# filixi/TCP-stack

Hardware: AMD Instinct MI355X
Metric: GiB/s device-resident TCP checksum over batched segments; % HBM roofline (higher is better)
Workload: dtype u16; 1 GPU; C2: 1M x 1460-B payload (1492-B images), fixed stride, device-resident; images_per_gpu=1048576, image_bytes=1492, bytes_per_gpu=1564475392, parallelism=shard1 (independent per-GPU batches, no collective)

## Files before the change

tcp-stack_amd/csrc/tcpck_device.h:

```cpp
#pragma once

#include <hip/hip_runtime.h>
#include <stdint.h>

#include "tcpck_internal.h"

namespace tcpck {
namespace dev {

using u32x4 = __attribute__((ext_vector_type(4))) unsigned int;

constexpr int kBlock = 256;
constexpr int kWavesPerBlock = kBlock / 64;

template <typename Kernel>
inline uint32_t resident_blocks_per_cu(Kernel kernel) {
  int nb = 0;
  if (hipOccupancyMaxActiveBlocksPerMultiprocessor(&nb, kernel, kBlock, 0) != hipSuccess || nb < 1) nb = 1;
  return static_cast<uint32_t>(nb);
}

inline uint32_t oversub_for(uint32_t requested, uint64_t bytes, uint64_t resident_waves, uint32_t max_m,
                            uint32_t min_run = 4u << 10) {
  if (requested) return requested;
  const uint64_t q = bytes / (resident_waves * min_run + 1);
  uint32_t m = 1;
  while (2 * m <= max_m && 2 * m <= q) m *= 2;
  return m;
}

__device__ __forceinline__ uint64_t align16_rel(const uint8_t *arena, uint64_t off) {
  const uint64_t mis = reinterpret_cast<uint64_t>(arena) & 15u;
  return ((off + mis) & ~uint64_t{15}) - mis;
}

__device__ __forceinline__ uint64_t align128_rel(const uint8_t *arena, uint64_t off) {
  const uint64_t mis = reinterpret_cast<uint64_t>(arena) & 127u;
  return ((off + mis) & ~uint64_t{127}) - mis;
}

__device__ __forceinline__ u32x4 load16_nt(const uint8_t *p) {
  return __builtin_nontemporal_load(reinterpret_cast<const u32x4 *>(p));
}

__device__ __forceinline__ uint32_t word_mask(int32_t lo, int32_t hi) {
  return ((1u << (hi >> 1)) - 1u) & ~((1u << (lo >> 1)) - 1u);
}

__device__ __forceinline__ uint32_t dword_mask(uint32_t wm, int j) {
  const uint32_t t = (wm >> (2 * j)) & 3u;
  return ((t & 1u) ? 0x0000FFFFu : 0u) | ((t & 2u) ? 0xFFFF0000u : 0u);
}

__device__ __forceinline__ u32x4 apply_mask(u32x4 w, uint32_t wm) {
  w.x &= dword_mask(wm, 0);
  w.y &= dword_mask(wm, 1);
  w.z &= dword_mask(wm, 2);
  w.w &= dword_mask(wm, 3);
  return w;
}

__device__ __forceinline__ uint32_t ref_add(uint32_t acc, uint32_t w) { return acc + w + (w >> 16); }

__device__ __forceinline__ uint32_t ref_chunk_sum(u32x4 w) {
  return ref_add(ref_add(ref_add(w.x + (w.x >> 16), w.y), w.z), w.w);
}

__device__ __forceinline__ uint32_t dot2_u16(uint32_t w, uint32_t acc) {
  uint32_t r;
  asm("v_dot2_u32_u16 %0, %1, %2, %3" : "=v"(r) : "v"(w), "s"(0x00010001u), "v"(acc));
  return r;
}
__device__ __forceinline__ uint32_t ref_chunk_sum_dot(u32x4 w) {
  return dot2_u16(w.w, dot2_u16(w.z, dot2_u16(w.y, dot2_u16(w.x, 0u))));
}

__device__ __forceinline__ __amdgpu_buffer_rsrc_t make_rsrc(const void *p, uint32_t bytes) {
  const uint64_t a = reinterpret_cast<uint64_t>(p);
  const uint32_t lo = static_cast<uint32_t>(__builtin_amdgcn_readfirstlane(static_cast<int>(a)));
  const uint32_t hi = static_cast<uint32_t>(__builtin_amdgcn_readfirstlane(static_cast<int>(a >> 32)));
  const int n = __builtin_amdgcn_readfirstlane(static_cast<int>(bytes));
  void *u = reinterpret_cast<void *>((static_cast<uint64_t>(hi) << 32) | lo);
  return __builtin_amdgcn_make_buffer_rsrc(u, 0, n, 0x00020000);
}
__device__ __forceinline__ void store16_field(__amdgpu_buffer_rsrc_t r, uint32_t voff, uint16_t v) {
  __builtin_amdgcn_raw_buffer_store_b16(v, r, static_cast<int>(voff), 0, 16);
}

__device__ __forceinline__ uint32_t n2h_selector(uint32_t j) {
  return j == 3 ? 0x02030001u : ((j == 2 || j >= 6) ? 0x02030100u : 0x00010203u);
}
__device__ __forceinline__ uint32_t n2h_dword(uint32_t h, uint32_t sel) {
  return __builtin_amdgcn_perm(h, h, sel);
}

__device__ __forceinline__ u32x4 load16_buf_nt(__amdgpu_buffer_rsrc_t r, uint32_t voff, uint32_t soff) {
  typedef unsigned v4u __attribute__((ext_vector_type(4)));
  const v4u v = __builtin_amdgcn_raw_buffer_load_b128(r, static_cast<int>(voff), static_cast<int>(soff), 2);
  return u32x4{v.x, v.y, v.z, v.w};
}

__device__ __forceinline__ uint32_t rfc_add(uint32_t acc, uint32_t w) {
  const uint32_t s = acc + w;
  return s + (s < w ? 1u : 0u);
}

template <int MODE>
__device__ __forceinline__ uint32_t accumulate(uint32_t acc, uint32_t w) {
  if constexpr (MODE == kRef) {
    return ref_add(acc, w);
  } else {
    return rfc_add(acc, w);
  }
}

template <int MODE>
__device__ __forceinline__ uint32_t fold_lane(uint32_t acc) {
  if constexpr (MODE == kRef) {
    return acc & 0xFFFFu;
  } else {
    acc = (acc & 0xFFFFu) + (acc >> 16);
    return (acc & 0xFFFFu) + (acc >> 16);
  }
}

template <int MODE>
__device__ __forceinline__ uint16_t finish(uint32_t sum) {
  if constexpr (MODE == kRef) {
    return static_cast<uint16_t>(~sum);
  } else {
    sum = (sum & 0xFFFFu) + (sum >> 16);
    sum = (sum & 0xFFFFu) + (sum >> 16);
    return static_cast<uint16_t>(~sum);
  }
}

template <int G>
__device__ __forceinline__ uint32_t group_sum(uint32_t x) {
#pragma unroll
  for (int m = G / 2; m >= 1; m >>= 1) x += __shfl_xor(x, m, 64);
  return x;
}

__device__ __forceinline__ uint32_t wave_inclusive_scan(uint32_t x) {
  x += __builtin_amdgcn_update_dpp(0, x, 0x111, 0xF, 0xF, false);
  x += __builtin_amdgcn_update_dpp(0, x, 0x112, 0xF, 0xF, false);
  x += __builtin_amdgcn_update_dpp(0, x, 0x114, 0xF, 0xF, false);
  x += __builtin_amdgcn_update_dpp(0, x, 0x118, 0xF, 0xF, false);
  x += __builtin_amdgcn_update_dpp(0, x, 0x142, 0xA, 0xF, false);
  x += __builtin_amdgcn_update_dpp(0, x, 0x143, 0xC, 0xF, false);
  return x;
}

__device__ __forceinline__ uint32_t read_lane(uint32_t x, uint32_t lane) {
  return static_cast<uint32_t>(__builtin_amdgcn_readlane(static_cast<int>(x), static_cast<int>(lane)));
}

__device__ __forceinline__ uint64_t read_lane64(uint64_t x, uint32_t lane) {
  const uint32_t lo = read_lane(static_cast<uint32_t>(x), lane);
  const uint32_t hi = read_lane(static_cast<uint32_t>(x >> 32), lane);
  return (static_cast<uint64_t>(hi) << 32) | lo;
}

template <bool EXACT = false>
__device__ __forceinline__ uint32_t words_before(uint32_t r, uint32_t x, uint32_t y, uint32_t z, uint32_t w) {
  const uint32_t nw = r >> 1;
  uint32_t h = 0;
  auto both = [](uint32_t d) -> uint32_t { return EXACT ? (d & 0xFFFFu) + (d >> 16) : d + (d >> 16); };
  if (nw >= 2) h += both(x);
  if (nw >= 4) h += both(y);
  if (nw >= 6) h += both(z);
  if (nw & 1) {
    const uint32_t d = nw == 1 ? x : (nw == 3 ? y : (nw == 5 ? z : w));
    h += d & 0xFFFFu;
  }
  return h;
}

template <int U, int MODE>
__device__ __forceinline__ uint32_t wave_image_sum(const uint8_t *arena, uint64_t start, uint32_t len,
                                                   bool exclude_field) {
  const uint32_t lane = threadIdx.x & 63;
  const uint64_t a0 = align16_rel(arena, start);
  const uint8_t *p0 = arena + a0;
  const int32_t lead = static_cast<int32_t>(start - a0);
  const int64_t span64 = lead + static_cast<int64_t>(len);
  const uint32_t nch = static_cast<uint32_t>((span64 + 15) >> 4);
  const int64_t field = exclude_field ? lead + 28 : -64;
  uint32_t acc = 0;
  for (uint32_t i0 = lane; i0 < nch; i0 += 64 * U) {
    u32x4 v[U];
#pragma unroll
    for (int u = 0; u < U; ++u) {
      const uint32_t i = i0 + u * 64;
      v[u] = load16_nt(p0 + 16 * static_cast<uint64_t>(i < nch ? i : nch - 1));
    }
#pragma unroll
    for (int u = 0; u < U; ++u) {
      const int64_t rel = 16 * static_cast<int64_t>(i0 + u * 64);
      const int32_t lo = static_cast<int32_t>(min(max(lead - rel, int64_t{0}), int64_t{16}));
      const int32_t hi = static_cast<int32_t>(min(max(span64 - rel, int64_t{0}), int64_t{16}));
      uint32_t wm = word_mask(lo, hi);
      const int64_t fb = field - rel;
      if (fb >= 0 && fb < 16) wm &= ~(1u << (fb >> 1));
      u32x4 w = v[u];
      if (wm != 0xFFu) w = apply_mask(w, wm);
      acc = accumulate<MODE>(acc, w.x);
      acc = accumulate<MODE>(acc, w.y);
      acc = accumulate<MODE>(acc, w.z);
      acc = accumulate<MODE>(acc, w.w);
    }
    if (MODE == kRfc1071) acc = fold_lane<MODE>(acc);
  }
  return group_sum<64>(fold_lane<MODE>(acc));
}

__device__ __forceinline__ uint64_t find_first_ge(const uint64_t *offsets, uint64_t base, uint64_t count, uint64_t target) {
  const uint32_t lane = threadIdx.x & 63;
  uint64_t lo = 0, hi = count;
  while (hi - lo > 64) {
    const uint64_t step = (hi - lo + 63) / 64;
    const uint64_t idx = lo + lane * step;
    const bool below = idx < hi && offsets[idx] - base < target;
    const uint32_t c = __popcll(__ballot(below));
    const uint64_t nlo = c ? lo + (c - 1) * step + 1 : lo;
    const uint64_t nhi = min(hi, lo + c * step);
    lo = nlo;
    hi = nhi;
  }
  const uint64_t idx = lo + lane;
  const bool below = idx < hi && offsets[idx] - base < target;
  return lo + __popcll(__ballot(below));
}

__device__ __forceinline__ void find_two(const uint64_t *offsets, uint64_t base, uint64_t count, uint64_t t0,
                                         uint64_t t1, uint64_t &r0, uint64_t &r1) {
  const uint32_t lane = threadIdx.x & 63;
  uint64_t lo[2] = {0, 0}, hi[2] = {count, count};
  const uint64_t t[2] = {t0, t1};
  while (hi[0] - lo[0] > 64 || hi[1] - lo[1] > 64) {
    uint64_t step[2], idx[2], v[2];
#pragma unroll
    for (int i = 0; i < 2; ++i) {
      step[i] = hi[i] - lo[i] > 64 ? (hi[i] - lo[i] + 63) / 64 : 1;
      idx[i] = lo[i] + lane * step[i];
      v[i] = idx[i] < hi[i] ? offsets[idx[i]] : 0;
    }
#pragma unroll
    for (int i = 0; i < 2; ++i) {
      if (hi[i] - lo[i] <= 64) continue;
      const bool below = idx[i] < hi[i] && v[i] - base < t[i];
      const uint32_t c = __popcll(__ballot(below));
      const uint64_t nlo = c ? lo[i] + (c - 1) * step[i] + 1 : lo[i];
      hi[i] = min(hi[i], lo[i] + c * step[i]);
      lo[i] = nlo;
    }
  }
  uint64_t v[2];
#pragma unroll
  for (int i = 0; i < 2; ++i) {
    const uint64_t idx = lo[i] + lane;
    v[i] = idx < hi[i] ? offsets[idx] : 0;
  }
  const bool b0 = lo[0] + lane < hi[0] && v[0] - base < t0;
  const bool b1 = lo[1] + lane < hi[1] && v[1] - base < t1;
  r0 = lo[0] + __popcll(__ballot(b0));
  r1 = lo[1] + __popcll(__ballot(b1));
}

__device__ __forceinline__ void count_split(uint64_t wid, uint64_t q, uint64_t r, uint64_t &kb, uint64_t &ke) {
  kb = wid * q + (wid < r ? wid : r);
  ke = kb + q + (wid < r ? 1u : 0u);
}

__device__ __forceinline__ uint32_t xcd_block(uint32_t b, uint32_t nb) {
  const uint32_t q = nb >> 3, r = nb & 7u, x = b & 7u;
  return (x < r ? x * (q + 1) : r * (q + 1) + (x - r) * q) + (b >> 3);
}

__device__ __forceinline__ uint32_t xcd_chunk_block(uint32_t b, uint32_t nb, uint32_t lc) {
  const uint32_t full = (nb >> (3 + lc)) << (3 + lc);
  if (b >= full) return b;
  const uint32_t i = b >> 3;
  return ((((i >> lc) << 3) + (b & 7u)) << lc) + (i & ((1u << lc) - 1u));
}

constexpr uint32_t kOrderDefault = 0xFFu;
constexpr uint32_t kOrderXcd = 0xFEu;
__device__ __forceinline__ uint32_t ordered_block(uint32_t b, uint32_t nb, uint32_t lc) {
  if (lc == kOrderDefault) return b;
  if (lc == kOrderXcd) return xcd_block(b, nb);
  return xcd_chunk_block(b, nb, lc);
}


}
}
```

tcp-stack_amd/csrc/tcpck_vvstream.hip:

```cpp
#include <type_traits>

#include "tcpck_device.h"
#include "tcpck_internal.h"

namespace tcpck {

namespace {

using dev::kBlock;
using dev::kWavesPerBlock;
using dev::u32x4;

constexpr uint32_t kRound = 256;
constexpr uint32_t kRing = 512;
constexpr uint32_t kMirror = 64;

struct VVArgs {
  uint8_t *arena;
  const uint64_t *offsets;
  const uint32_t *lengths;
  uint64_t base;
  uint64_t count;
  void *out;
  uint64_t per_wave, rem;
  uint32_t stride;
  uint32_t len;
  uint32_t order;
  uint32_t keep_first;
  uint32_t defer_field;
  uint64_t *dbg;
};

#ifdef TCPCK_PROBE
__device__ __forceinline__ uint64_t stamp_after(uint32_t dep) {
  uint64_t t;
  asm volatile("s_memrealtime %0\n\ts_waitcnt lgkmcnt(0)" : "=s"(t) : "v"(dep));
  return t;
}
#endif

__device__ __forceinline__ u32x4 zero_word(u32x4 w, uint32_t wi) {
  const uint32_t keep = (wi & 1u) ? 0x0000FFFFu : 0xFFFF0000u;
  const uint32_t di = wi >> 1;
  w.x &= di == 0 ? keep : 0xFFFFFFFFu;
  w.y &= di == 1 ? keep : 0xFFFFFFFFu;
  w.z &= di == 2 ? keep : 0xFFFFFFFFu;
  w.w &= di == 3 ? keep : 0xFFFFFFFFu;
  return w;
}

[[maybe_unused]] __device__ __forceinline__ u32x4 put_word(u32x4 w, uint32_t wi, uint32_t v) {
  const uint32_t sh = (wi & 1u) << 4;
  const uint32_t m = ~(0xFFFFu << sh), x = (v & 0xFFFFu) << sh;
  const uint32_t di = wi >> 1;
  w.x = di == 0 ? (w.x & m) | x : w.x;
  w.y = di == 1 ? (w.y & m) | x : w.y;
  w.z = di == 2 ? (w.z & m) | x : w.z;
  w.w = di == 3 ? (w.w & m) | x : w.w;
  return w;
}

[[maybe_unused]] __device__ __forceinline__ void store16_chunk_wt(__amdgpu_buffer_rsrc_t r, uint32_t voff, u32x4 v) {
  typedef unsigned v4u __attribute__((ext_vector_type(4)));
  __builtin_amdgcn_raw_buffer_store_b128(v4u{v.x, v.y, v.z, v.w}, r, static_cast<int>(voff), 0, 19);
}

template <int U, int OP, int SPLIT, int LAYOUT, bool KEEP = false, int MODE = kRef, bool BLK = false>
__global__ void __launch_bounds__(kBlock) vvstream_kernel(VVArgs a) {
  constexpr bool FIXED = LAYOUT != 0;
  constexpr bool GAP = LAYOUT == 2;
  static_assert(!BLK || (OP == kFill && !GAP && MODE == kRef && !KEEP), "BLK: reference-mode FILL, no gaps");
  constexpr uint32_t kMinFill = BLK ? 64u : 30u;
  __shared__ u32x4 s_blk[kWavesPerBlock][BLK ? 4 : 1];
  __shared__ uint32_t s_end[kWavesPerBlock][FIXED ? 1 : kRing + kMirror];
  __shared__ __attribute__((aligned(16))) uint32_t s_pre[kWavesPerBlock][MODE == kRef ? 256 : 512];
  __shared__ uint32_t s_fld[kWavesPerBlock][OP == kFill ? 64 : 1];
  const uint32_t lane = threadIdx.x & 63;
  const uint32_t wv = static_cast<uint32_t>(__builtin_amdgcn_readfirstlane(static_cast<int>(threadIdx.x >> 6)));
  const uint64_t W = static_cast<uint64_t>(gridDim.x) * kWavesPerBlock;
  const uint32_t bid = dev::ordered_block(blockIdx.x, gridDim.x, a.order);
  const uint64_t wid = static_cast<uint64_t>(bid) * kWavesPerBlock + wv;
  const uint64_t N = a.count;
#ifdef TCPCK_PROBE
  const uint64_t t_start = a.dbg ? __builtin_amdgcn_s_memrealtime() : 0;
  uint64_t t_desc = 0, t_first = 0;
#endif
  const uint32_t S = a.stride;
  const uint32_t L = FIXED ? a.len : 0u;
  uint64_t kb, ke;
  if (FIXED || SPLIT == 1) {
    dev::count_split(wid, a.per_wave, a.rem, kb, ke);
  } else {
    const uint64_t first = a.offsets[0] - a.base;
    const uint64_t total = a.offsets[N - 1] - a.base + a.lengths[N - 1] - first;
    const uint64_t q = total / W, rm = total % W;
    dev::find_two(a.offsets, a.base, N, first + q * wid + rm * wid / W,
                  first + q * (wid + 1) + rm * (wid + 1) / W, kb, ke);
    if (wid == 0) kb = 0;
    if (wid + 1 == W) ke = N;
  }
  if (kb >= ke) return;

  uint64_t s0, s1;
  if constexpr (FIXED) {
    s0 = kb * S;
    s1 = (ke - 1) * S + L;
  } else {
    s0 = a.offsets[kb] - a.base;
    s1 = a.offsets[ke - 1] - a.base + a.lengths[ke - 1];
  }
  uint8_t *const arena = a.arena;
  const uint64_t A0 = dev::align128_rel(arena, s0);
  const uint32_t nimg = static_cast<uint32_t>(ke - kb);
  const uint32_t nv = GAP ? 2 * nimg : nimg;
  bool bad = !(s1 >= s0 && s1 - A0 < (uint64_t{1} << 31));
#ifdef TCPCK_PROBE
  if (a.dbg) t_desc = stamp_after(static_cast<uint32_t>(s1 - A0));
#endif

  auto store = [&](uint64_t k, uint32_t sum, uint64_t start) {
    const uint16_t c = dev::finish<MODE>(sum);
    if constexpr (OP == kVerify) {
      static_cast<uint8_t *>(a.out)[k] = (c == 0) ? 1 : 0;
    } else {
      if (a.out) static_cast<uint16_t *>(a.out)[k] = c;
      if (OP == kFill) *reinterpret_cast<uint16_t *>(arena + start + 28) = c;
    }
  };
  auto store_rel = [&](uint64_t k, uint32_t sum, uint32_t start_rel, __amdgpu_buffer_rsrc_t r) {
    const uint16_t c = dev::finish<MODE>(sum);
    if constexpr (OP == kVerify) {
      static_cast<uint8_t *>(a.out)[k] = (c == 0) ? 1 : 0;
    } else {
      if (a.out) static_cast<uint16_t *>(a.out)[k] = c;
      if (OP == kFill && !a.defer_field) dev::store16_field(r, start_rel + 28, c);
    }
  };

  if (!bad) {
    const uint32_t lead = static_cast<uint32_t>(s0 - A0);
    const uint32_t span = static_cast<uint32_t>(s1 - A0);
    const uint32_t nsteps = (span + 1023) >> 10;
    const uint32_t last_chunk = span > 0 ? (span - 1) >> 4 : 0;
    int64_t blo = 0, bhi = 0;
    uint32_t extent = (last_chunk + 1) << 4;
    if constexpr (BLK) {
      const uint64_t b0 = FIXED ? 0 : a.offsets[0] - a.base;
      const uint64_t b1 = FIXED ? (N - 1) * S + L : a.offsets[N - 1] - a.base + a.lengths[N - 1];
      blo = static_cast<int64_t>(b0) - static_cast<int64_t>(A0);
      bhi = static_cast<int64_t>(b1) - static_cast<int64_t>(A0);
      const int64_t want = min(static_cast<int64_t>((span + 63u) & ~63u), bhi & ~int64_t{15});
      if (want > static_cast<int64_t>(extent)) extent = static_cast<uint32_t>(want);
    }
    const auto rsrc = dev::make_rsrc(arena + A0, extent);
    auto whole = [&](uint32_t b) { return static_cast<int64_t>(b) >= blo && static_cast<int64_t>(b) + 64 <= bhi; };
    uint32_t stage_f = 0;
    auto load_step = [&](uint32_t st) -> u32x4 {
      if constexpr (KEEP) {
        typedef unsigned v4u __attribute__((ext_vector_type(4)));
        const v4u v = __builtin_amdgcn_raw_buffer_load_b128(rsrc, static_cast<int>(lane << 4), static_cast<int>(st << 10), 0);
        return u32x4{v.x, v.y, v.z, v.w};
      } else {
        return dev::load16_buf_nt(rsrc, lane << 4, st << 10);
      }
    };
    uint32_t *ring_end = s_end[wv];
    u32x4 *pre4 = reinterpret_cast<u32x4 *>(s_pre[wv]);
    const uint16_t *pre16 = reinterpret_cast<const uint16_t *>(s_pre[wv]);
    uint32_t *fld = s_fld[wv];
    if constexpr (OP == kFill) {
      fld[lane] = 0;
      __builtin_amdgcn_wave_barrier();
    }

    uint32_t carry = 0, p_last = 0, jn = 0, fj = 0;
    uint32_t e_last = lead;
    u32x4 ring[U];
#pragma unroll
    for (int u = 0; u < U; ++u) {
      if (u == 0 && a.keep_first && (lane < 8 || a.keep_first == 2)) {
        typedef unsigned v4u __attribute__((ext_vector_type(4)));
        const v4u v = __builtin_amdgcn_raw_buffer_load_b128(rsrc, static_cast<int>(lane << 4), 0, 0);
        ring[0] = u32x4{v.x, v.y, v.z, v.w};
      } else {
        ring[u] = load_step(static_cast<uint32_t>(u));
      }
    }

    const uint32_t *lens = FIXED ? nullptr : a.lengths + kb;
    auto load_round = [&](uint32_t r, uint32_t (&d)[4]) {
#pragma unroll
      for (int i = 0; i < 4; ++i) {
        const uint32_t j = r * kRound + 4 * lane + i;
        d[i] = j < nimg ? lens[j] : 0u;
      }
    };
    uint32_t loaded = FIXED ? nv : 0;
    uint32_t pos = lead;
    bool short_fill = false;
    bool al4 = (lead & 3u) == 0 && (!FIXED || ((S & 3u) == 0 && (!GAP || (L & 3u) == 0)));
    auto fill_round = [&]() {
      const uint32_t r = loaded / kRound;
      uint32_t d[4];
      load_round(r, d);
      al4 = al4 && __ballot(((d[0] | d[1] | d[2] | d[3]) & 3u) != 0) == 0;
      if constexpr (MODE == kRfc1071) {
        bad = bad || __ballot((d[0] | d[1] | d[2] | d[3]) >= (1u << 17)) != 0;
      }
      const uint32_t e1 = d[0], e2 = e1 + d[1], e3 = e2 + d[2], e4 = e3 + d[3];
      const uint32_t incl = dev::wave_inclusive_scan(e4);
      const uint32_t ex = pos + incl - e4;
      if constexpr (OP == kFill) {
        const uint32_t jb = r * kRound + 4 * lane;
        bool sh = false;
#pragma unroll
        for (int i = 0; i < 4; ++i) sh |= (jb + i < nimg) && d[i] < kMinFill;
        short_fill |= __ballot(sh) != 0;
      }
      const uint32_t jb = r * kRound + 4 * lane;
      const uint32_t v0 = jb < nimg ? ex + e1 : ~0u, v1 = jb + 1 < nimg ? ex + e2 : ~0u;
      const uint32_t v2 = jb + 2 < nimg ? ex + e3 : ~0u, v3 = jb + 3 < nimg ? ex + e4 : ~0u;
      const uint32_t si = (r * kRound) % kRing + 4 * lane;
      ring_end[si] = v0;
      ring_end[si + 1] = v1;
      ring_end[si + 2] = v2;
      ring_end[si + 3] = v3;
      if (si < kMirror) {
        ring_end[kRing + si] = v0;
        ring_end[kRing + si + 1] = v1;
        ring_end[kRing + si + 2] = v2;
        ring_end[kRing + si + 3] = v3;
      }
      pos = pos + dev::read_lane(incl, 63);
      loaded += kRound;
      if (loaded >= nimg) {
        const uint32_t sn = loaded % kRing + lane;
        ring_end[sn] = ~0u;
        if (sn < kMirror) ring_end[kRing + sn] = ~0u;
      }
      __builtin_amdgcn_wave_barrier();
    };
    if constexpr (!FIXED) {
      fill_round();
      if constexpr (OP == kFill) {
        if (nimg > kRound) {
          uint32_t sum = 0;
          bool sh = false;
          for (uint32_t j = lane; j < nimg; j += 64) {
            const uint32_t l = lens[j];
            sum += l;
            sh |= l < kMinFill || (MODE == kRfc1071 && l >= (1u << 17));
          }
          short_fill = short_fill || __ballot(sh) != 0;
          bad = bad || short_fill || lead + dev::group_sum<64>(sum) != span;
        } else {
          bad = bad || short_fill || pos != span;
        }
      }
    } else {
      if constexpr (OP == kFill) bad = L < kMinFill;
    }
    auto end_of = [&](uint32_t j) -> uint32_t {
      if constexpr (GAP) {
        return lead + (j >> 1) * S + (j & 1u) * L;
      } else if constexpr (FIXED) {
        return lead + (j + 1) * S;
      } else {
        return ring_end[j % kRing];
      }
    };
    auto ends_at = [&](uint32_t jn0) -> uint32_t {
      if constexpr (FIXED) {
        const uint32_t j = jn0 + lane;
        return j < nv ? end_of(j) : ~0u;
      } else {
        return ring_end[jn0 % kRing + lane];
      }
    };

    auto stream_run = [&](auto al4_tag) {
      constexpr bool AL4 = decltype(al4_tag)::value;
      for (uint32_t g = 0; g < nsteps && !bad; g += U) {
  #pragma unroll
        for (int u = 0; u < U; ++u) {
          const uint32_t st = g + u;
          const uint32_t sb = st << 10;
          const uint32_t c = sb + (lane << 4);
          u32x4 w = ring[u];
          const u32x4 raw = w;
          if (sb == 0 || sb + 1024 > span) {
            const int32_t lo = min(max(static_cast<int32_t>(lead) - static_cast<int32_t>(c), 0), 16);
            const int32_t hi = min(max(static_cast<int32_t>(span) - static_cast<int32_t>(c), 0), 16);
            w = dev::apply_mask(w, dev::word_mask(lo, hi));
          }
          if (!FIXED && jn + 66 > loaded && loaded < nimg) fill_round();
          uint32_t j = jn + lane;
          uint32_t e = ends_at(jn);
          if constexpr (OP == kFill) {
            const uint32_t i = fj + lane;
            uint32_t f;
            if constexpr (FIXED)
              f = lead + i * S + 28;
            else
              f = (i == 0 ? lead : (i < nimg ? end_of(i - 1) : span)) + 28;
            const bool inf = i < nimg && f < sb + 1024;
            const uint64_t bf = __ballot(inf);
            if (bf) {
              if (inf) fld[(f - sb) >> 4] = ((f & 15u) >> 1) + 1u;
              __builtin_amdgcn_wave_barrier();
              const uint32_t q = fld[lane];
              if (q) {
                fld[lane] = 0u;
                w = zero_word(w, q - 1u);
              }
              __builtin_amdgcn_wave_barrier();
              fj += static_cast<uint32_t>(__popcll(bf));
            }
          }
          const uint32_t q1 = dev::dot2_u16(w.x, 0u);
          const uint32_t q2 = dev::dot2_u16(w.y, q1);
          const uint32_t q3 = dev::dot2_u16(w.z, q2);
          const uint32_t tot = dev::dot2_u16(w.w, q3);
#ifdef TCPCK_PROBE
          if (a.dbg && st == 0) t_first = stamp_after(tot);
#endif
          const uint32_t incl = dev::wave_inclusive_scan(tot);
          bool table = false;
          for (;;) {
            const bool inb = e < sb + 1024;
            const uint64_t bal = __ballot(inb);
            if (!bal) break;
            if (!table) {
              const uint32_t p0 = carry + incl - tot;
              const uint32_t b1 = p0 + q1, b2 = p0 + q2, b3 = p0 + q3;
              if constexpr (AL4) {
                pre4[lane] = u32x4{p0, b1, b2, b3};
              } else if constexpr (MODE == kRfc1071) {
                pre4[2 * lane] = u32x4{p0, p0 + (w.x & 0xFFFFu), b1, b1 + (w.y & 0xFFFFu)};
                pre4[2 * lane + 1] = u32x4{b2, b2 + (w.z & 0xFFFFu), b3, b3 + (w.w & 0xFFFFu)};
              } else
                pre4[lane] = u32x4{__builtin_amdgcn_perm(p0 + w.x, p0, 0x05040100u),
                                   __builtin_amdgcn_perm(b1 + w.y, b1, 0x05040100u),
                                   __builtin_amdgcn_perm(b2 + w.z, b2, 0x05040100u),
                                   __builtin_amdgcn_perm(b3 + w.w, b3, 0x05040100u)};
              __builtin_amdgcn_wave_barrier();
              table = true;
            }
            const uint32_t cnt = static_cast<uint32_t>(__popcll(bal));
            const uint32_t off = min(e - sb, 1022u);
            const uint32_t P = AL4 ? s_pre[wv][off >> 2]
                                   : (MODE == kRfc1071 ? s_pre[wv][off >> 1] : static_cast<uint32_t>(pre16[off >> 1]));
            const uint32_t pprev = static_cast<uint32_t>(
                __builtin_amdgcn_update_dpp(static_cast<int>(p_last), static_cast<int>(P), 0x138, 0xF, 0xF, false));
            if constexpr (OP == kFill) {
              const uint32_t el = static_cast<uint32_t>(
                  __builtin_amdgcn_update_dpp(static_cast<int>(e_last), static_cast<int>(e), 0x138, 0xF, 0xF, false));
              const uint32_t start = lane == 0 ? e_last : el;
              if constexpr (BLK) {
                if (inb) {
                  const uint16_t c = dev::finish<MODE>(P - pprev);
                  if (a.out) static_cast<uint16_t *>(a.out)[kb + j] = c;
                  const uint32_t f = start + 28;
                  if (f >= sb) {
                    fld[(f - sb) >> 4] = 0x80000000u | (((f & 15u) >> 1) << 16) | c;
                  } else if (whole(f & ~63u)) {
                    reinterpret_cast<uint16_t *>(s_blk[wv])[(f & 63u) >> 1] = c;
                  } else {
                    dev::store16_field(rsrc, f, c);
                  }
                }
              } else if (inb && (!GAP || (j & 1u))) {
                store_rel(kb + (GAP ? j >> 1 : j), P - pprev, start, rsrc);
              }
            } else {
              if (inb && (!GAP || (j & 1u))) store(kb + (GAP ? j >> 1 : j), P - pprev, 0);
            }
            p_last = dev::read_lane(P, cnt - 1);
            e_last = dev::read_lane(e, cnt - 1);
            jn += cnt;
            if (cnt < 64) break;
            if (!FIXED && jn + 66 > loaded && loaded < nimg) fill_round();
            j = jn + lane;
            e = ends_at(jn);
          }
          if constexpr (BLK) {
            __builtin_amdgcn_wave_barrier();
            if (stage_f != 0 && stage_f < e_last) {
              if (lane < 4 && whole(stage_f & ~63u)) store16_chunk_wt(rsrc, (stage_f & ~63u) + 16 * lane, s_blk[wv][lane]);
              stage_f = 0;
            }
            const uint32_t v = fld[lane];
            const uint64_t bv = __ballot(v != 0);
            if (bv) {
              const uint32_t cb = sb + ((lane & ~3u) << 4);
              if ((bv >> (lane & ~3u)) & 0xFull) {
                if (whole(cb))
                  store16_chunk_wt(rsrc, sb + (lane << 4), v ? put_word(raw, (v >> 16) & 7u, v) : raw);
                else if (v)
                  dev::store16_field(rsrc, sb + (lane << 4) + (((v >> 16) & 7u) << 1), static_cast<uint16_t>(v));
              }
              if (v) fld[lane] = 0u;
            }
            if (jn < nv) {
              const uint32_t f = e_last + 28;
              if (f >= sb && f < sb + 1024) {
                const uint32_t cb = f & ~63u;
                if (((sb + (lane << 4)) & ~63u) == cb) s_blk[wv][lane & 3u] = raw;
                stage_f = f;
              }
            }
          }
          __builtin_amdgcn_wave_barrier();
          carry += dev::read_lane(incl, 63);
          ring[u] = load_step(st + U);
        }
      }
    };
    if (al4 && (FIXED || loaded >= nimg))
      stream_run(std::true_type{});
    else
      stream_run(std::false_type{});
    if constexpr (!FIXED) bad = bad || pos != span || loaded < nimg;
    if (BLK && !bad && jn < nv) {
      const uint16_t c = dev::finish<MODE>(carry - p_last);
      if (lane == 0 && a.out) static_cast<uint16_t *>(a.out)[kb + jn] = c;
      const uint32_t f = e_last + 28;
      if (whole(f & ~63u)) {
        if (lane == 0) reinterpret_cast<uint16_t *>(s_blk[wv])[(f & 63u) >> 1] = c;
        __builtin_amdgcn_wave_barrier();
        if (lane < 4) store16_chunk_wt(rsrc, (f & ~63u) + 16 * lane, s_blk[wv][lane]);
      } else if (lane == 0) {
        dev::store16_field(rsrc, f, c);
      }
      jn = nv - 1 == jn ? nv : jn;
    }
    if (!bad && jn < nv) {
      const uint32_t rem = nv - jn;
      for (uint32_t i = lane; i < rem; i += 64) {
        const uint32_t v = jn + i;
        if (!GAP || (v & 1u)) store_rel(kb + (GAP ? v >> 1 : v), i == 0 ? carry - p_last : 0u, i == 0 ? e_last : span, rsrc);
      }
      jn = nv;
    }
    bad = bad || jn != nv;
  }
#ifdef TCPCK_PROBE
  if (a.dbg && lane == 0) {
    uint32_t hw_id, xcc_id;
    asm volatile("s_getreg_b32 %0, hwreg(HW_REG_HW_ID)" : "=s"(hw_id));
    asm volatile("s_getreg_b32 %0, hwreg(HW_REG_XCC_ID)" : "=s"(xcc_id));
    uint64_t *d = a.dbg + 8 * wid;
    d[0] = t_start;
    d[1] = t_desc;
    d[2] = t_first;
    d[3] = __builtin_amdgcn_s_memrealtime();
    d[4] = hw_id | (static_cast<uint64_t>(xcc_id) << 32);
    d[5] = ke - kb;
    d[6] = s1 - s0;
    d[7] = 0;
  }
#endif
  if (bad) {
    for (uint64_t k = kb; k < ke; ++k) {
      const uint64_t start = FIXED ? k * S : a.offsets[k] - a.base;
      const uint32_t len = FIXED ? L : a.lengths[k];
      if (OP == kFill && len < 30) continue;
      const uint32_t sum = dev::wave_image_sum<2, MODE>(arena, start, len, OP == kFill);
      if (lane == 0) store(k, sum, start);
    }
  }
}

template <int U, int OP, int SPLIT, int LAYOUT, bool KEEP = false, int MODE = kRef, bool BLK = false>
hipError_t launch_one(const RunArgs &s, uint32_t oversub, int flags, uint32_t num_cus, hipStream_t stream) {
  static const uint32_t per_cu = dev::resident_blocks_per_cu(vvstream_kernel<U, OP, SPLIT, LAYOUT, KEEP, MODE, BLK>);
  const uint64_t resident = static_cast<uint64_t>(per_cu) * num_cus;
  uint64_t blocks = resident * (oversub ? oversub : 1);
  const uint64_t need = (s.count + kWavesPerBlock - 1) / kWavesPerBlock;
  if (blocks > need) blocks = need;
  if (blocks == 0) return hipSuccess;
  VVArgs a{};
  a.arena = s.arena;
  a.offsets = s.offsets;
  a.lengths = s.lengths;
  a.base = s.base;
  a.count = s.count;
  a.out = s.out;
  a.per_wave = s.count / (blocks * kWavesPerBlock);
  a.rem = s.count % (blocks * kWavesPerBlock);
  a.stride = static_cast<uint32_t>(s.stride);
  a.len = s.len;
  a.order = (flags & 8) ? 4u : dev::kOrderDefault;
  a.keep_first = (flags & 16) ? ((flags & 256) ? 2u : 1u) : 0u;
  a.defer_field = (flags & 64) ? 1u : 0u;
  a.dbg = s.dbg;
  hipLaunchKernelGGL((vvstream_kernel<U, OP, SPLIT, LAYOUT, KEEP, MODE, BLK>), dim3(static_cast<uint32_t>(blocks)),
                     dim3(kBlock), 0, stream, a);
  return hipGetLastError();
}

template <int U, int SPLIT, int LAYOUT>
hipError_t dispatch(int op, const RunArgs &a, uint32_t oversub, int flags, uint32_t num_cus, hipStream_t s) {
  if (a.mode != kRef) {
    switch (op) {
      case kChecksum: return launch_one<U, kChecksum, SPLIT, LAYOUT, false, kRfc1071>(a, oversub, flags, num_cus, s);
      case kVerify: return launch_one<U, kVerify, SPLIT, LAYOUT, false, kRfc1071>(a, oversub, flags, num_cus, s);
      case kFill: return launch_one<U, kFill, SPLIT, LAYOUT, false, kRfc1071>(a, oversub, flags, num_cus, s);
      default: return hipErrorInvalidValue;
    }
  }
  switch (op) {
    case kChecksum: return launch_one<U, kChecksum, SPLIT, LAYOUT>(a, oversub, flags, num_cus, s);
    case kVerify: return launch_one<U, kVerify, SPLIT, LAYOUT>(a, oversub, flags, num_cus, s);
    case kFill:
#ifdef TCPCK_PROBE
      if constexpr (LAYOUT != 2)
        if (flags & 128) return launch_one<U, kFill, SPLIT, LAYOUT, false, kRef, true>(a, oversub, flags, num_cus, s);
#endif
      return (flags & 32) ? launch_one<U, kFill, SPLIT, LAYOUT, true>(a, oversub, flags, num_cus, s)
                          : launch_one<U, kFill, SPLIT, LAYOUT>(a, oversub, flags, num_cus, s);
    default: return hipErrorInvalidValue;
  }
}

}

hipError_t launch_vvstream(int op, int variant, bool fixed, const RunArgs &a, uint32_t num_cus,
                           hipStream_t stream) {
  if (a.count == 0) return hipSuccess;
  if (fixed && (a.len == 0 || a.stride < a.len || a.stride > (1u << 24))) return hipErrorInvalidValue;
  const bool gap = fixed && a.stride != a.len;
  const uint64_t bytes = fixed ? a.count * a.stride : a.total_bytes;
  uint32_t m = a.oversub ? a.oversub : 1;
  int flags = variant & 248;
  if ((flags & 64) && (op != kFill || !a.out)) return hipErrorInvalidValue;
#ifdef TCPCK_PROBE
  if ((flags & 128) && (op != kFill || a.mode != kRef || gap || (flags & 96))) return hipErrorInvalidValue;
#else
  if (flags & 128) return hipErrorInvalidValue;
#endif
  variant &= 7;
#ifdef TCPCK_PROBE
  if (variant == 5) {
    variant = 4;
    flags |= 256;
  }
#endif
  int u8 = (variant & 1);
  int split = variant >= 2 ? 1 : 0;
  if (variant == 4) {
    m = dev::oversub_for(a.oversub, bytes, static_cast<uint64_t>(num_cus) * 32, 1024, 8u << 10);
    u8 = m >= 32;
    if (op == kFill && !fixed && !(flags & 224)) {
      m = dev::oversub_for(a.oversub, bytes, static_cast<uint64_t>(num_cus) * 32, 1024, 4u << 10);
      u8 = false;
    }
    split = m >= 4;
  } else {
#ifdef TCPCK_PROBE
    if (variant > 4 || variant < 0) return hipErrorInvalidValue;
#else
    return hipErrorInvalidValue;
#endif
  }
  if (gap) return u8 ? dispatch<8, 1, 2>(op, a, m, flags, num_cus, stream) : dispatch<4, 1, 2>(op, a, m, flags, num_cus, stream);
  if (fixed) return u8 ? dispatch<8, 1, 1>(op, a, m, flags, num_cus, stream) : dispatch<4, 1, 1>(op, a, m, flags, num_cus, stream);
  if (split) return u8 ? dispatch<8, 1, 0>(op, a, m, flags, num_cus, stream) : dispatch<4, 1, 0>(op, a, m, flags, num_cus, stream);
  return u8 ? dispatch<8, 0, 0>(op, a, m, flags, num_cus, stream) : dispatch<4, 0, 0>(op, a, m, flags, num_cus, stream);
}

}
```

Measured before the change: 6912 GiB/s.

## Unify AL4 stream loop, precompute prefix table terms, issue next load early

Merges the two template-specialized stream_run lambdas into a single loop with a runtime AL4 flag. For kRef mode it precomputes per-chunk packed partial sums before the scan and builds the prefix table with packed u16 adds. In non-BLK kRef mode it issues the next ring load right after the chunk sum instead of at the end of the step. It also forces the U=4 unroll in place of U=8 for large oversubscription. Together these aim to cut instruction count and code size and to overlap memory latency. The cost is a runtime branch on AL4, and the smaller unroll gives less memory parallelism.

```diff
diff --git a/tcp-stack_amd/csrc/tcpck_device.h b/tcp-stack_amd/csrc/tcpck_device.h
--- a/tcp-stack_amd/csrc/tcpck_device.h
+++ b/tcp-stack_amd/csrc/tcpck_device.h
@@ -70,6 +70,10 @@
   uint32_t r;
   asm("v_dot2_u32_u16 %0, %1, %2, %3" : "=v"(r) : "v"(w), "s"(0x00010001u), "v"(acc));
   return r;
+}
+__device__ __forceinline__ uint32_t pk_add_u16(uint32_t a, uint32_t b) {
+  typedef unsigned short u16x2 __attribute__((ext_vector_type(2)));
+  return __builtin_bit_cast(uint32_t, static_cast<u16x2>(__builtin_bit_cast(u16x2, a) + __builtin_bit_cast(u16x2, b)));
 }
 __device__ __forceinline__ uint32_t ref_chunk_sum_dot(u32x4 w) {
   return dot2_u16(w.w, dot2_u16(w.z, dot2_u16(w.y, dot2_u16(w.x, 0u))));
diff --git a/tcp-stack_amd/csrc/tcpck_vvstream.hip b/tcp-stack_amd/csrc/tcpck_vvstream.hip
--- a/tcp-stack_amd/csrc/tcpck_vvstream.hip
+++ b/tcp-stack_amd/csrc/tcpck_vvstream.hip
@@ -1,5 +1,3 @@
-#include <type_traits>
-
 #include "tcpck_device.h"
 #include "tcpck_internal.h"
 
@@ -278,8 +276,10 @@
       }
     };
 
-    auto stream_run = [&](auto al4_tag) {
-      constexpr bool AL4 = decltype(al4_tag)::value;
+    {
+      const bool AL4 = al4 && (FIXED || loaded >= nimg);
+      constexpr bool PRE = MODE == kRef;
+      constexpr bool EARLY = PRE && !BLK;
       for (uint32_t g = 0; g < nsteps && !bad; g += U) {
   #pragma unroll
         for (int u = 0; u < U; ++u) {
@@ -321,6 +321,14 @@
           const uint32_t q2 = dev::dot2_u16(w.y, q1);
           const uint32_t q3 = dev::dot2_u16(w.z, q2);
           const uint32_t tot = dev::dot2_u16(w.w, q3);
+          uint32_t r0, r1, r2, r3;
+          if (PRE && !AL4) {
+            r0 = w.x << 16;
+            r1 = __builtin_amdgcn_perm(q1 + w.y, q1, 0x05040100u);
+            r2 = __builtin_amdgcn_perm(q2 + w.z, q2, 0x05040100u);
+            r3 = __builtin_amdgcn_perm(q3 + w.w, q3, 0x05040100u);
+          }
+          if constexpr (EARLY) ring[u] = load_step(st + U);
 #ifdef TCPCK_PROBE
           if (a.dbg && st == 0) t_first = stamp_after(tot);
 #endif
@@ -333,23 +341,25 @@
             if (!table) {
               const uint32_t p0 = carry + incl - tot;
               const uint32_t b1 = p0 + q1, b2 = p0 + q2, b3 = p0 + q3;
-              if constexpr (AL4) {
+              if (AL4) {
                 pre4[lane] = u32x4{p0, b1, b2, b3};
+                asm volatile("");
               } else if constexpr (MODE == kRfc1071) {
                 pre4[2 * lane] = u32x4{p0, p0 + (w.x & 0xFFFFu), b1, b1 + (w.y & 0xFFFFu)};
                 pre4[2 * lane + 1] = u32x4{b2, b2 + (w.z & 0xFFFFu), b3, b3 + (w.w & 0xFFFFu)};
-              } else
-                pre4[lane] = u32x4{__builtin_amdgcn_perm(p0 + w.x, p0, 0x05040100u),
-                                   __builtin_amdgcn_perm(b1 + w.y, b1, 0x05040100u),
-                                   __builtin_amdgcn_perm(b2 + w.z, b2, 0x05040100u),
-                                   __builtin_amdgcn_perm(b3 + w.w, b3, 0x05040100u)};
+              } else {
+                asm volatile("" : "+v"(r0), "+v"(r1), "+v"(r2), "+v"(r3));
+                const uint32_t pp = __builtin_amdgcn_perm(p0, p0, 0x05040100u);
+                pre4[lane] = u32x4{dev::pk_add_u16(r0, pp), dev::pk_add_u16(r1, pp), dev::pk_add_u16(r2, pp),
+                                   dev::pk_add_u16(r3, pp)};
+              }
               __builtin_amdgcn_wave_barrier();
               table = true;
             }
             const uint32_t cnt = static_cast<uint32_t>(__popcll(bal));
             const uint32_t off = min(e - sb, 1022u);
-            const uint32_t P = AL4 ? s_pre[wv][off >> 2]
-                                   : (MODE == kRfc1071 ? s_pre[wv][off >> 1] : static_cast<uint32_t>(pre16[off >> 1]));
+            const uint32_t P =
+                MODE == kRfc1071 ? s_pre[wv][off >> (AL4 ? 2 : 1)] : static_cast<uint32_t>(pre16[off >> 1]);
             const uint32_t pprev = static_cast<uint32_t>(
                 __builtin_amdgcn_update_dpp(static_cast<int>(p_last), static_cast<int>(P), 0x138, 0xF, 0xF, false));
             if constexpr (OP == kFill) {
@@ -412,14 +422,10 @@
           }
           __builtin_amdgcn_wave_barrier();
           carry += dev::read_lane(incl, 63);
-          ring[u] = load_step(st + U);
+          if constexpr (!EARLY) ring[u] = load_step(st + U);
         }
       }
-    };
-    if (al4 && (FIXED || loaded >= nimg))
-      stream_run(std::true_type{});
-    else
-      stream_run(std::false_type{});
+    }
     if constexpr (!FIXED) bad = bad || pos != span || loaded < nimg;
     if (BLK && !bad && jn < nv) {
       const uint16_t c = dev::finish<MODE>(carry - p_last);
@@ -550,10 +556,9 @@
   int split = variant >= 2 ? 1 : 0;
   if (variant == 4) {
     m = dev::oversub_for(a.oversub, bytes, static_cast<uint64_t>(num_cus) * 32, 1024, 8u << 10);
-    u8 = m >= 32;
+    u8 = false;
     if (op == kFill && !fixed && !(flags & 224)) {
       m = dev::oversub_for(a.oversub, bytes, static_cast<uint64_t>(num_cus) * 32, 1024, 4u << 10);
-      u8 = false;
     }
     split = m >= 4;
   } else {
```

After: 6890 GiB/s. About the same (-0.3%).
